# rubiruchi/ofdm_uhd

Hardware: AMD Instinct MI355X
Metric: OFDM symbols/sec (TX+loopback RX) @ N_fft=512; packet CRC pass rate (higher is better)
Workload: dtype f32; 1 GPU; N_fft=512, occ=200, QPSK, CP=128, synthetic AWGN channel (BASELINE configs[1]); payload_bytes=1026, symbols_per_packet=22, streams=1, iq_buffers=1, parallelism=independent streams, 1 per GPU

## Files before the change

ofdm_uhd_amd/csrc/engine_rx.inc:

```

template <typename T>
static int dev_excl_scan(ofdm_handle* h, const T* d_in, uint64_t n, T* d_out, T* d_total) {
  const uint64_t nb = (n + SCAN_BLOCK - 1) / SCAN_BLOCK;
  HIPCHK(h, h->rx.partial.ensure(sizeof(T) * std::max<uint64_t>(nb, 1)));
  T* part = h->rx.partial.as<T>();
  if (n == 0) {
    if (d_total) HIPCHK(h, hipMemsetAsync(d_total, 0, sizeof(T), h->stream));
    return OFDM_OK;
  }
  hipLaunchKernelGGL(HIP_KERNEL_NAME(k_scan_partials<T>), dim3((unsigned)nb), dim3(256), 0, h->stream, d_in, n, part);
  hipLaunchKernelGGL(HIP_KERNEL_NAME(k_scan_top<T>), dim3(1), dim3(256), 0, h->stream, part, nb, d_total);
  hipLaunchKernelGGL(HIP_KERNEL_NAME(k_scan_final<T>), dim3((unsigned)nb), dim3(256), 0, h->stream, d_in, n, part, d_out);
  HIPCHK(h, hipGetLastError());
  return OFDM_OK;
}

template <int N, bool TWL, bool TAPS, bool CSI = false>
static int launch_demod_t(ofdm_handle* h, const DemodParams& q, size_t shmem) {
  constexpr int T = N / 8, FPW = demod_fpw(N);
  if (shmem > 64 * 1024)
    HIPCHK(h, hipFuncSetAttribute(reinterpret_cast<const void*>(&k_rx_demod<N, TWL, TAPS, CSI>),
                                  hipFuncAttributeMaxDynamicSharedMemorySize, (int)shmem));
  hipLaunchKernelGGL(HIP_KERNEL_NAME(k_rx_demod<N, TWL, TAPS, CSI>), dim3((q.nframes + FPW - 1) / FPW), dim3(T * FPW), shmem,
                     h->stream, q);
  HIPCHK(h, hipGetLastError());
  return OFDM_OK;
}
template <int N, bool TWL>
static int launch_demod_v(ofdm_handle* h, const DemodParams& q, size_t shmem) {
  if (q.csi_eq) return launch_demod_t<N, TWL, true, true>(h, q, shmem);
  const bool instr = q.tap_mode != 0 || q.tap_sampler || q.tap_fft || q.tap_acq || q.tap_sink || q.tap_demapped || q.qual;
  return instr ? launch_demod_t<N, TWL, true>(h, q, shmem) : launch_demod_t<N, TWL, false>(h, q, shmem);
}

template <int N>
static int launch_demod(ofdm_handle* h, const DemodParams& q0) {
  DemodParams q = q0;
  constexpr int T = N / 8, WAVES = demod_fpw(N) * ((T + WAVE - 1) / WAVE);
  const bool grid = q.grid != nullptr;
  const bool csi = q.csi_eq != nullptr;
  auto bytes = [&](bool twl, bool sm) {
    return (size_t)demod_lds_bytes(N, twl, sm, q.occ, q.arity, q.nmap, q.nbits, q.shift, grid, csi);
  };
  constexpr int CU_WAVES = 4 * demod_waves_per_simd(N);
  auto wgs = [&](size_t b) { return std::max<size_t>(1, std::min<size_t>(std::max(1, CU_WAVES / WAVES), CU_LDS_BYTES / b)); };
  constexpr bool base_twl = !fft_onebuf(N);
  const size_t w0 = wgs(bytes(base_twl, false));
  bool twl = base_twl;
  if constexpr (fft_onebuf(N)) twl = wgs(bytes(true, false)) == w0 && bytes(true, false) <= CU_LDS_BYTES;
  q.smap_lds = (wgs(bytes(twl, true)) == w0 && bytes(twl, true) <= CU_LDS_BYTES) ? 1 : 0;
  if (const char* e = getenv("OFDM_DEMOD_LDS")) {
    const int v = atoi(e);
    if constexpr (fft_onebuf(N)) twl = (v & 1) != 0;
    q.smap_lds = (v >> 1) & 1;
  }
  const size_t shmem = bytes(twl, q.smap_lds != 0);
  if (shmem > CU_LDS_BYTES) FAIL(h, OFDM_E_INVAL, "configuration needs more than 160 KiB of LDS in k_rx_demod");
  if constexpr (fft_onebuf(N)) {
    return twl ? launch_demod_v<N, true>(h, q, shmem) : launch_demod_v<N, false>(h, q, shmem);
  } else {
    return launch_demod_v<N, true>(h, q, shmem);
  }
}

static int run_demod(ofdm_handle* h, const DemodParams& q) {
  switch (h->N) {
    case 64: return launch_demod<64>(h, q);
    case 128: return launch_demod<128>(h, q);
    case 256: return launch_demod<256>(h, q);
    case 512: return launch_demod<512>(h, q);
    case 1024: return launch_demod<1024>(h, q);
    case 2048: return launch_demod<2048>(h, q);
    default: return launch_demod<4096>(h, q);
  }
}

enum { CT_CAND = 0, CT_OVERFLOW = 1, CT_NLO = 2, CT_NHI = 3, CT_CHAIN = 4, CT_NPEAKS = 5, CT_NSYM = 6, CT_KEYTOT = 7,
       CT_DEFR = 8 , CT_RAWTOT = 13, CT_PIECES = 14, CT_STASH = 15, CT_RECS = 16, CT_COUNT = 17 };

static int sync_params(ofdm_handle* h, uint64_t nsamples, bool cap_full, SyncParams* out) {
  RxState& rx = h->rx;
  const int N = h->N, CP = h->CP, T = SYNC_TILE;
  const uint64_t ntiles = (nsamples + T - 1) / T;
  const int tiles_per_seg = 32 * ((N + CP + T - 1) / T);
  const uint64_t egrid = std::min<uint64_t>(ntiles, 256ull * 8ull), egrid_small = std::min<uint64_t>(ntiles, 256ull * 16ull);
  const uint64_t cand_cap = (cap_full ? nsamples + nsamples / 8 : nsamples / 16) + (egrid + 16) * SYNC_CHUNK_C + egrid_small * 2048ull;
  const uint64_t piece_cap = (cap_full ? nsamples / 2 + 1 : nsamples / 128) + (egrid + egrid_small + 16) * SYNC_CHUNK_P;
  HIPCHK(h, rx.y.ensure(nsamples * sizeof(c32)));
  HIPCHK(h, rx.tile_B.ensure(ntiles * sizeof(double)));
  HIPCHK(h, rx.tile_np.ensure(ntiles * sizeof(uint32_t)));
  HIPCHK(h, rx.tile_pieces.ensure(piece_cap * sizeof(SyncPiece)));
  HIPCHK(h, rx.tile_first.ensure(ntiles * sizeof(uint64_t)));
  HIPCHK(h, rx.avg_in.ensure(ntiles * sizeof(double)));
  HIPCHK(h, rx.cand_u.ensure(cand_cap * sizeof(float)));
  HIPCHK(h, rx.cand_P.ensure(cand_cap * sizeof(c32)));
  HIPCHK(h, rx.counters.ensure(CT_COUNT * sizeof(uint64_t)));
  HIPCHK(h, rx.counts.ensure(ntiles * sizeof(uint32_t)));
  HIPCHK(h, rx.offsets.ensure(ntiles * sizeof(uint32_t)));
  HIPCHK(h, rx.recs.ensure(ntiles * sizeof(SyncRec)));
  float *d_metric = nullptr, *d_presel = nullptr;
  if (h->tap_mask & (1u << OFDM_TAP_RX_METRIC)) {
    HIPCHK(h, rx.metric.ensure(nsamples * sizeof(float)));
    d_metric = rx.metric.as<float>();
  }
  if (h->tap_mask & (1u << OFDM_TAP_RX_PRESEL)) {
    HIPCHK(h, rx.presel.ensure(nsamples * sizeof(float)));
    d_presel = rx.presel.as<float>();
  }
  uint64_t* ctr = rx.counters.as<uint64_t>();
  SyncParams sp;
  memset(&sp, 0, sizeof(sp));
  sp.N = N;
  sp.D = N / 2;
  sp.CP = CP;
  sp.HY = (N + 7) / 8 * 8;
  sp.HM = CP;
  sp.R = sync_ring_samples(sp.HY);
  sp.tiles_per_seg = tiles_per_seg;
  sp.nsamples = nsamples;
  sp.ntiles = ntiles;
  sp.tapcp = (float)(1.0 / (double)CP);
  sp.cand_thr = -fmaxf(h->cfg.peak_rise, h->cfg.peak_fall);
  sp.alpha = h->cfg.peak_alpha;
  sp.decay = (double)(1.0f - h->cfg.peak_alpha);
  sp.y = rx.y.as<c32>();
  sp.metric_tap = d_metric;
  sp.presel_tap = d_presel;
  sp.dpow = h->d_synctab.as<double>();
  sp.ipow = sp.dpow + (SYNC_TILE + 1);
  sp.wtab = reinterpret_cast<const float*>(sp.ipow + (SYNC_TILE + 1));
  sp.tile_B = rx.tile_B.as<double>();
  sp.tile_npieces = rx.tile_np.as<uint32_t>();
  sp.tile_first = rx.tile_first.as<uint64_t>();
  sp.pieces = rx.tile_pieces.as<SyncPiece>();
  sp.piece_cap = piece_cap;
  sp.piece_count = reinterpret_cast<unsigned long long*>(ctr + CT_PIECES);
  sp.cand_u = rx.cand_u.as<float>();
  sp.cand_P = rx.cand_P.as<c32>();
  sp.cand_cap = cand_cap;
  sp.cand_count = reinterpret_cast<unsigned long long*>(ctr + CT_CAND);
  sp.overflow = reinterpret_cast<unsigned int*>(ctr + CT_OVERFLOW);
  sp.recs = rx.recs.as<SyncRec>();
  sp.rec_count = reinterpret_cast<unsigned long long*>(ctr + CT_RECS);
  sp.exact_small = sync_exact_small(CP, N / 2);
  if (const char* es = getenv("OFDM_EXACT_SMALL")) sp.exact_small = std::max(0, std::min(atoi(es), (int)SYNC_TILE));
#ifdef SYNC_DIAG
  if (const char* ab = getenv("OFDM_ABLATE")) sp.ablate = atoi(ab);
#endif
  if (sp.HM > T) FAIL(h, OFDM_E_INVAL, "cyclic prefix longer than a k_sync tile");
  *out = sp;
  return OFDM_OK;
}

static uint64_t sync_nseg(const SyncParams& sp) { return (sp.ntiles + (uint64_t)sp.tiles_per_seg - 1) / (uint64_t)sp.tiles_per_seg; }

#ifdef SYNC_STAMPS
static DevBuf g_stamp_buf;
static int stamps_prepare(ofdm_handle* h, SyncParams& sp, uint64_t nseg) {
  HIPCHK(h, g_stamp_buf.ensure(nseg * 16 * sizeof(unsigned long long)));
  HIPCHK(h, hipMemsetAsync(g_stamp_buf.p, 0, nseg * 16 * sizeof(unsigned long long), h->stream));
  sp.stamps = g_stamp_buf.as<unsigned long long>();
  return OFDM_OK;
}
static int sync_stamps_report(ofdm_handle* h, const unsigned long long* d_stamps, uint64_t nseg, int tiles_per_seg) {
  HIPCHK(h, hipStreamSynchronize(h->stream));
  std::vector<unsigned long long> st(nseg * 16);
  HIPCHK(h, hipMemcpy(st.data(), d_stamps, st.size() * 8, hipMemcpyDeviceToHost));
  double sum[16] = {0};
  for (uint64_t i = 0; i < nseg; i++)
    for (int k = 0; k < 16; k++) sum[k] += (double)st[i * 16 + k];
  const char* nm[16] = {"-", "y tile -> ring / filter", "B2 wait", "terms", "scan3 (B3)", "M + B4", "mavg + B5", "summary", "filter: block A", "filter: block B", "filter: taps + windows in", "-", "-", "-", "-", "-"};
  double tot = 0;
  for (int k = 0; k < 16; k++) tot += sum[k];
  fprintf(stderr, "[k_sync stamps] %llu workgroups, s_memtime ticks per workgroup-tile (wave 0):\n", (unsigned long long)nseg);
  for (int k = 0; k < 11; k++)
    fprintf(stderr, "  %-26s %10.0f  %5.1f%%\n", nm[k], sum[k] / (double)nseg / (double)(tiles_per_seg + 1), 100.0 * sum[k] / tot);
  return OFDM_OK;
}
#endif

static bool front_fused(const ofdm_handle* h) {
  if (h->cfg.sync_mode != OFDM_SYNC_PN) return false;
  const char* e = getenv("OFDM_FRONT");
  if (!e || atoi(e) == 0) return false;
  const int F = h->filtF, B = F - (int)h->cfg.ntaps + 1;
  if (F > 512) return false;
  const int HY = (h->N + 7) / 8 * 8, C = (B + 7) / 8 * 8;
  if (HY + C > SYNC_TILE || h->CP > SYNC_TILE) return false;
  return front_lds_layout(sync_ring_samples(HY), h->CP, B, F).total <= CU_LDS_BYTES / 3;
}

static int launch_sync(ofdm_handle* h, SyncParams& sp) {
  RxState& rx = h->rx;
  const int T = SYNC_TILE;
  const uint64_t nseg = sync_nseg(sp);
  HIPCHK(h, hipMemsetAsync(rx.counters.p, 0, CT_COUNT * sizeof(uint64_t), h->stream));
#ifdef SYNC_STAMPS
  if (int rs = stamps_prepare(h, sp, nseg)) return rs;
#endif
  const size_t sync_shmem = sync_lds_layout(sp.R, sp.HM).total;
  if (sync_shmem > CU_LDS_BYTES) FAIL(h, OFDM_E_INVAL, "configuration needs more than 160 KiB of LDS in k_sync");
  {
    ProfScope span(h->prof, OFDM_K_SYNC, h->stream);
    int wg = (int)std::min<size_t>(SYNC_MAX_WG, CU_LDS_BYTES / sync_shmem);
    if (const char* w = getenv("OFDM_SYNC_W")) wg = std::min(wg, atoi(w));
    bool fixed_layout = sp.R - (int)T <= (int)T;
    if (const char* e = getenv("OFDM_SYNC_STATIC")) fixed_layout = fixed_layout && (atoi(e) != 0 || sync_mt_overlay(sp.R));
    const void* fn = fixed_layout ? (wg >= 6   ? reinterpret_cast<const void*>(&k_sync<6, true>)
                                     : wg == 5 ? reinterpret_cast<const void*>(&k_sync<5, true>)
                                     : wg == 4 ? reinterpret_cast<const void*>(&k_sync<4, true>)
                                     : wg == 3 ? reinterpret_cast<const void*>(&k_sync<3, true>)
                                               : reinterpret_cast<const void*>(&k_sync<2, true>))
                                  : (wg >= 4   ? reinterpret_cast<const void*>(&k_sync<4, false>)
                                     : wg == 3 ? reinterpret_cast<const void*>(&k_sync<3, false>)
                                               : reinterpret_cast<const void*>(&k_sync<2, false>));
    HIPCHK(h, hipFuncSetAttribute(fn, hipFuncAttributeMaxDynamicSharedMemorySize, (int)sync_shmem));
    FilterParams nofp;
    memset(&nofp, 0, sizeof(nofp));
    void* args[] = {&sp, &nofp};
    HIPCHK(h, hipLaunchKernel(fn, dim3((unsigned)nseg), dim3(SYNC_THREADS), args, sync_shmem, h->stream));
  }
  HIPCHK(h, hipGetLastError());
  return OFDM_OK;
}

static void rx_note_input(ofdm_handle* h, const ofdm_c32* iq, uint64_t nsamples) {
  std::swap(h->ev_rx_in, h->ev_rx_in_old);
  h->rx_in_old_pending = h->rx_in_pending;
  h->rx_in_lo[1] = h->rx_in_lo[0];
  h->rx_in_hi[1] = h->rx_in_hi[0];
  h->rx_in_lo[0] = (uintptr_t)iq;
  h->rx_in_hi[0] = (uintptr_t)iq + nsamples * rx_ss(h);
}

static int launch_front(ofdm_handle* h, FilterParams& fp, uint64_t nsamples) {
  const int F = h->filtF;
  SyncParams sp;
  int rcs = sync_params(h, nsamples, false, &sp);
  if (rcs != OFDM_OK) return rcs;
  HIPCHK(h, hipMemsetAsync(h->rx.counters.p, 0, CT_COUNT * sizeof(uint64_t), h->stream));
  const size_t shm = front_lds_layout(sp.R, sp.HM, fp.B, F).total;
  const uint64_t nseg = sync_nseg(sp);
  const void* fn = F == 64    ? reinterpret_cast<const void*>(&k_sync<3, true, 64>)
                   : F == 128 ? reinterpret_cast<const void*>(&k_sync<3, true, 128>)
                   : F == 256 ? reinterpret_cast<const void*>(&k_sync<3, true, 256>)
                              : reinterpret_cast<const void*>(&k_sync<3, true, 512>);
  HIPCHK(h, hipFuncSetAttribute(fn, hipFuncAttributeMaxDynamicSharedMemorySize, (int)shm));
#ifdef SYNC_STAMPS
  if (int rs = stamps_prepare(h, sp, nseg)) return rs;
#endif
  void* args[] = {&sp, &fp};
  {
    ProfScope span(h->prof, OFDM_K_FRONT, h->stream);
    HIPCHK(h, hipLaunchKernel(fn, dim3((unsigned)nseg), dim3(SYNC_THREADS), args, shm, h->stream));
  }
  HIPCHK(h, hipGetLastError());
#ifdef SYNC_STAMPS
  if (int rs = sync_stamps_report(h, sp.stamps, nseg, sp.tiles_per_seg)) return rs;
#endif
  h->rx.front_done = true;
  return OFDM_OK;
}

template <typename XT>
static int launch_filter_t(ofdm_handle* h, FilterParams& fp, uint64_t nsamples) {
  const int F = h->filtF;
  const uint64_t bpr = 256 / (F / 8);
  const uint64_t nblk = (nsamples + (uint64_t)fp.goff + (uint64_t)fp.B - 1) / (uint64_t)fp.B;
  fp.nrounds = (nblk + bpr - 1) / bpr;
  const size_t fsh = (size_t)256 * 9 * sizeof(c32);
  const unsigned fgrid = (unsigned)std::min<uint64_t>(fp.nrounds, 256ull * 8ull * 4ull);
  {
    ProfScope span(h->prof, OFDM_K_FILTER, h->stream);
    switch (F) {
      case 64: hipLaunchKernelGGL(HIP_KERNEL_NAME(k_chan_filter<64, XT>), dim3(fgrid), dim3(256), fsh, h->stream, fp); break;
      case 128: hipLaunchKernelGGL(HIP_KERNEL_NAME(k_chan_filter<128, XT>), dim3(fgrid), dim3(256), fsh, h->stream, fp); break;
      case 256: hipLaunchKernelGGL(HIP_KERNEL_NAME(k_chan_filter<256, XT>), dim3(fgrid), dim3(256), fsh, h->stream, fp); break;
      case 512: hipLaunchKernelGGL(HIP_KERNEL_NAME(k_chan_filter<512, XT>), dim3(fgrid), dim3(256), fsh, h->stream, fp); break;
      case 1024: hipLaunchKernelGGL(HIP_KERNEL_NAME(k_chan_filter<1024, XT>), dim3(fgrid), dim3(256), fsh, h->stream, fp); break;
      default: FAIL(h, OFDM_E_INVAL, "unsupported channel filter transform length");
    }
  }
  HIPCHK(h, hipGetLastError());
  return OFDM_OK;
}

static int launch_filter(ofdm_handle* h, FilterParams& fp, uint64_t nsamples) {
  return h->rx_fmt == OFDM_IQ_SC16 ? launch_filter_t<sc16>(h, fp, nsamples) : launch_filter_t<c32>(h, fp, nsamples);
}

static int rx_submit_impl(ofdm_handle* h, const ofdm_c32* iq, uint64_t nsamples, const c32** d_x_out) {
  RxState& rx = h->rx;
  HIPCHK(h, hipSetDevice(h->cfg.device_id));
  if (h->tx_pending && h->txs != h->stream) HIPCHK(h, hipStreamWaitEvent(h->stream, h->ev_tx_done, 0));
  h->tx_pending = false;
  const c32* d_x = reinterpret_cast<const c32*>(iq);
  if (h->rx_fmt == OFDM_IQ_SC16) {
    if ((uintptr_t)iq & 3u) FAIL(h, OFDM_E_INVAL, "ofdm_sc16 buffers must be 4-byte aligned");
    if (front_fused(h)) FAIL(h, OFDM_E_INVAL, "the fused front end (OFDM_FRONT=1) takes float32 samples only");
  }
  if (!h->dev_ptrs) {
    HIPCHK(h, rx.x_stage.ensure(nsamples * rx_ss(h)));
    HIPCHK(h, hipMemcpyAsync(rx.x_stage.p, iq, nsamples * rx_ss(h), hipMemcpyHostToDevice, h->stream));
    d_x = rx.x_stage.as<c32>();
  }
  *d_x_out = d_x;
  rx.in_event_at_end = true;
  if (h->cfg.sync_mode != OFDM_SYNC_PN) return OFDM_OK;
  HIPCHK(h, rx.y.ensure(nsamples * sizeof(c32)));
  FilterParams fp;
  memset(&fp, 0, sizeof(fp));
  fp.B = h->filtF - (int)h->cfg.ntaps + 1;
  fp.ntm1 = (int)h->cfg.ntaps - 1;
  fp.goff = (int)(rx.origin % (uint64_t)fp.B);
  fp.nsamples = nsamples;
  fp.x = d_x;
  fp.y = rx.y.as<c32>();
  fp.Hf = h->d_Hf.as<c32>();
  fp.twF = h->d_twF.as<c32>();
  fp.xscale = h->rx_scale;
  rx.front_done = false;
  if (int rc = front_fused(h) ? launch_front(h, fp, nsamples) : launch_filter(h, fp, nsamples)) return rc;
  if (!h->sense.rx_on) {
    rx_note_input(h, iq, nsamples);
    HIPCHK(h, hipEventRecord(h->ev_rx_in, h->stream));
    h->rx_in_pending = true;
    rx.in_event_at_end = false;
  }
  return OFDM_OK;
}

extern "C" int ofdm_rx_submit(ofdm_handle* h, const ofdm_c32* iq, uint64_t nsamples) {
  if (!h) return OFDM_E_INVAL;
  if (nsamples && !iq) FAIL(h, OFDM_E_INVAL, "null argument");
  RxState& rx = h->rx;
  rx.sub_valid = false;
  if (nsamples == 0) return OFDM_OK;
  const c32* d_x = nullptr;
  int rc = rx_submit_impl(h, iq, nsamples, &d_x);
  if (rc != OFDM_OK) return rc;
  rx.sub_valid = true;
  rx.sub_iq = iq;
  rx.sub_n = nsamples;
  rx.sub_dx = d_x;
  rx.sub_hold = rx.in_event_at_end;
  return OFDM_OK;
}

struct RxCall {
  ofdm_handle* h;
  const ofdm_c32* iq;
  uint64_t nsamples;
  uint8_t* payload_out;
  uint64_t payload_cap;
  uint64_t* payload_off;
  uint32_t* payload_len;
  uint8_t* crc_ok;
  int max_pkts;
  int* npkt;
  ofdm_stats* stats;
  const c32* d_x = nullptr;
  bool fixed = false;
  bool done = false;
  bool dyn = false;
  uint64_t npeaks = 0, nforced = 0;
  uint64_t n_lo = 0, nframes = 0, nsym = 0, npk = 0, nbytes = 0, rawtot = 0;
  uint64_t npk_ub = 0;
  DynFrames dynf;
  DemodParams dq;
  DeframeParams fq;
  CsiRows csi_fr = {nullptr, nullptr, nullptr, nullptr};
  uint8_t* d_pay = nullptr;
};

static uint64_t* rx_ctr(ofdm_handle* h) { return h->rx.counters.as<uint64_t>(); }

static int rx_read_counts(RxCall& c) {
  ofdm_handle* h = c.h;
  RxState& rx = h->rx;
  uint64_t hc[CT_COUNT];
  HIPCHK(h, hipMemcpyAsync(hc, rx.counters.p, sizeof(hc), hipMemcpyDeviceToHost, h->stream));
  HIPCHK(h, hipStreamSynchronize(h->stream));
  c.n_lo = hc[CT_NLO] & 0xFFFFFFFFull;
  c.nframes = c.npeaks - c.n_lo - (hc[CT_NHI] & 0xFFFFFFFFull);
  c.nsym = hc[CT_NSYM];
  c.npk = hc[CT_KEYTOT] >> 40;
  c.nbytes = hc[CT_KEYTOT] & ((1ull << 40) - 1);
  c.rawtot = hc[CT_RAWTOT];
  rx.nframes = c.nframes;
  rx.j0 = c.n_lo;
  rx.nsym_total = c.nsym;
  if (c.stats) {
    c.stats->frames = c.nframes;
    c.stats->symbols = c.nsym;
    c.stats->headers_ok = hc[CT_DEFR + 0];
    c.stats->chained_frames = hc[CT_DEFR + 3];
    c.stats->overflow = hc[CT_OVERFLOW] & 0xFFFFFFFFull;
  }
  return OFDM_OK;
}

static int rx_check_capacity(RxCall& c) {
  if (c.npk <= (uint64_t)c.max_pkts && c.nbytes <= c.payload_cap) return OFDM_OK;
  *c.npkt = (int)std::min<uint64_t>(c.npk, 0x7FFFFFFF);
  FAIL(c.h, OFDM_E_CAPACITY, "payload_out / max_pkts too small for the packets found");
}

static hipError_t launch_sync_exact(const void* fn, unsigned grid, size_t shmem, SyncParams sp, hipStream_t s) {
  void* args[] = {&sp};
  return hipLaunchKernel(fn, dim3(grid), dim3(SYNC_THREADS), args, shmem, s);
}

static int rx_sync_exact(RxCall& c, SyncParams& sp, bool cap_full) {
  ofdm_handle* h = c.h;
  if (cap_full) {
    int rcs = sync_params(h, c.nsamples, true, &sp);
    if (rcs != OFDM_OK) return rcs;
    uint64_t* ctr = rx_ctr(h);
    HIPCHK(h, hipMemsetAsync(ctr + CT_CAND, 0, 2 * sizeof(uint64_t), h->stream));
    HIPCHK(h, hipMemsetAsync(ctr + CT_NPEAKS, 0, sizeof(uint64_t), h->stream));
    HIPCHK(h, hipMemsetAsync(ctr + CT_PIECES, 0, 2 * sizeof(uint64_t), h->stream));
  }
  const unsigned egrid = (unsigned)std::min<uint64_t>(sp.ntiles, 256ull * 8ull);
  const unsigned egrid_small = (unsigned)std::min<uint64_t>(sp.ntiles, 256ull * 16ull);
  {
    ProfScope span(h->prof, OFDM_K_EXACT, h->stream);
    const size_t esh = exact_lds_layout(sp.CP, SYNC_TILE).total, esh_small = exact_lds_layout(sp.CP, sp.exact_small).total;
    const void* fbig = sp.D >= 2048 ? reinterpret_cast<const void*>(&k_sync_exact<SYNC_THREADS, true>)
                                    : reinterpret_cast<const void*>(&k_sync_exact<SYNC_THREADS, false>);
    if (esh > 64 * 1024) HIPCHK(h, hipFuncSetAttribute(fbig, hipFuncAttributeMaxDynamicSharedMemorySize, (int)esh));
    if (sp.exact_small > 0)
      hipLaunchKernelGGL(HIP_KERNEL_NAME(k_sync_exact<WAVE, false>), dim3(egrid_small), dim3(WAVE), esh_small, h->stream, sp);
    HIPCHK(h, launch_sync_exact(fbig, egrid, esh, sp, h->stream));
    if (sp.metric_tap) {
      SyncParams tp = sp;
      tp.tap_only = 1;
      HIPCHK(h, launch_sync_exact(fbig, egrid, esh, tp, h->stream));
    }
  }
  HIPCHK(h, hipGetLastError());
#ifdef SYNC_STAMPS
  if (!h->rx.front_done)
    if (int rs = sync_stamps_report(h, sp.stamps, sync_nseg(sp), sp.tiles_per_seg)) return rs;
#endif
  return OFDM_OK;
}

static int rx_sense_fork(RxCall& c) {
  ofdm_handle* h = c.h;
  SenseState& ss = h->sense;
  HIPCHK(h, hipEventRecord(ss.ev_in, h->stream));
  HIPCHK(h, hipStreamWaitEvent(ss.side, ss.ev_in, 0));
  int src = sense_enqueue(h, &ss.rx_cfg, c.d_x, c.nsamples, ss.side);
  if (src != OFDM_OK) return src;
  HIPCHK(h, hipEventRecord(ss.ev_out, ss.side));
  return OFDM_OK;
}

static PeakParams make_peak_params(ofdm_handle* h, const SyncParams& sp) {
  RxState& rx = h->rx;
  PeakParams pp;
  memset(&pp, 0, sizeof(pp));
  pp.ntiles = sp.ntiles;
  pp.nsamples = sp.nsamples;
  pp.rise = h->cfg.peak_rise;
  pp.fall = h->cfg.peak_fall;
  pp.alpha = h->cfg.peak_alpha;
  pp.dpow = sp.dpow;
  pp.tile_npieces = rx.tile_np.as<uint32_t>();
  pp.tile_first = rx.tile_first.as<uint64_t>();
  pp.pieces = rx.tile_pieces.as<SyncPiece>();
  pp.avg_in = rx.avg_in.as<double>();
  pp.cand_u = rx.cand_u.as<float>();
  pp.cand_P = rx.cand_P.as<c32>();
  pp.counts = rx.counts.as<uint32_t>();
  pp.offsets = rx.offsets.as<uint32_t>();
  pp.stash_peaks = rx.stash_peaks.as<uint64_t>();
  pp.stash_P = rx.stash_P.as<c32>();
  pp.stash_overflow = reinterpret_cast<unsigned int*>(rx_ctr(h) + CT_STASH);
  if (h->tap_mask & (1u << OFDM_TAP_RX_RUN_AVG)) pp.run_rows = rx.run_rows.as<double>();
  return pp;
}

static int rx_flags_pn(RxCall& c, const SyncParams& sp, uint64_t* overflow) {
  ofdm_handle* h = c.h;
  RxState& rx = h->rx;
  const uint64_t ntiles = sp.ntiles;
  const unsigned grid = (unsigned)((ntiles + 255) / 256);
  uint64_t* ctr = rx_ctr(h);
  const uint64_t run_cap = (h->tap_mask & (1u << OFDM_TAP_RX_RUN_AVG)) ? sp.piece_cap : 0;
  HIPCHK(h, rx.stash_peaks.ensure(ntiles * PEAK_STASH * sizeof(uint64_t)));
  HIPCHK(h, rx.stash_P.ensure(ntiles * PEAK_STASH * sizeof(c32)));
  if (run_cap) HIPCHK(h, rx.run_rows.ensure(run_cap * 2 * sizeof(double)));
  PeakParams pp = make_peak_params(h, sp);
  hipLaunchKernelGGL(k_avg_carry, dim3(grid), dim3(256), 0, h->stream, rx.tile_B.as<double>(), ntiles, c.nsamples, sp.dpow,
                     rx.avg_in.as<double>());
  if (run_cap) HIPCHK(h, hipMemsetAsync(rx.run_rows.p, 0xFF, run_cap * 2 * sizeof(double), h->stream));
  hipLaunchKernelGGL(HIP_KERNEL_NAME(k_peak<false>), dim3(grid), dim3(256), 0, h->stream, pp);
  HIPCHK(h, hipGetLastError());
  int rc = dev_excl_scan<uint32_t>(h, rx.counts.as<uint32_t>(), ntiles, rx.offsets.as<uint32_t>(),
                                   reinterpret_cast<uint32_t*>(ctr + CT_NPEAKS));
  if (rc) return rc;
  uint64_t hc[CT_COUNT];
  HIPCHK(h, hipMemcpyAsync(hc, ctr, sizeof(hc), hipMemcpyDeviceToHost, h->stream));
  HIPCHK(h, hipStreamSynchronize(h->stream));
  if ((*overflow = hc[CT_OVERFLOW] & 0xFFFFFFFFull)) return OFDM_OK;
  rx.run_slots = std::min<uint64_t>(hc[CT_PIECES], run_cap);
  const uint64_t npeaks = hc[CT_NPEAKS] & 0xFFFFFFFFull;
  c.npeaks = rx.npeaks = npeaks;
  if (c.stats) c.stats->peaks = npeaks;
  if (npeaks == 0 && !(rx.nco_ref_on && !rx.hist_flags.empty())) {
    c.done = true;
    return OFDM_OK;
  }
  HIPCHK(h, rx.peaks.ensure(std::max<uint64_t>(npeaks, 1) * sizeof(uint64_t)));
  HIPCHK(h, rx.peak_P.ensure(std::max<uint64_t>(npeaks, 1) * sizeof(c32)));
  pp.peaks = rx.peaks.as<uint64_t>();
  pp.peak_P = rx.peak_P.as<c32>();
  if (npeaks > 0) {
    if (hc[CT_STASH] & 0xFFFFFFFFull)
      hipLaunchKernelGGL(HIP_KERNEL_NAME(k_peak<true>), dim3(grid), dim3(256), 0, h->stream, pp);
    else
      hipLaunchKernelGGL(k_peak_compact, dim3(grid), dim3(256), 0, h->stream, pp);
    HIPCHK(h, hipGetLastError());
  }
  return OFDM_OK;
}

__global__ void __launch_bounds__(256) k_fixed_flags(uint64_t npeaks, uint64_t first, uint64_t period, uint64_t* __restrict__ peaks,
                                                      c32* __restrict__ peak_P) {
  const uint64_t k = (uint64_t)blockIdx.x * blockDim.x + threadIdx.x;
  if (k >= npeaks) return;
  peaks[k] = first + k * period;
  peak_P[k] = mk(0.f, 0.f);
}

static int rx_fixed_count(RxCall& c) {
  ofdm_handle* h = c.h;
  RxState& rx = h->rx;
  const uint64_t L = (uint64_t)h->L;
  c.npeaks = rx.npeaks = c.nsamples >= L ? (c.nsamples - L) / ((uint64_t)h->cfg.fixed_nsymbols * L) + 1 : 0;
  if (c.stats) c.stats->peaks = c.npeaks;
  HIPCHK(h, rx.counters.ensure(CT_COUNT * sizeof(uint64_t)));
  HIPCHK(h, hipMemsetAsync(rx.counters.p, 0, CT_COUNT * sizeof(uint64_t), h->stream));
  if (c.npeaks == 0) {
    HIPCHK(h, hipStreamSynchronize(h->stream));
    c.done = true;
  }
  return OFDM_OK;
}

static int rx_flags_fixed(RxCall& c) {
  ofdm_handle* h = c.h;
  RxState& rx = h->rx;
  HIPCHK(h, rx.peaks.ensure(c.npeaks * sizeof(uint64_t)));
  HIPCHK(h, rx.peak_P.ensure(c.npeaks * sizeof(c32)));
  hipLaunchKernelGGL(k_fixed_flags, dim3((unsigned)((c.npeaks + 255) / 256)), dim3(256), 0, h->stream, c.npeaks, (uint64_t)h->L - 1,
                     (uint64_t)h->cfg.fixed_nsymbols * (uint64_t)h->L, rx.peaks.as<uint64_t>(), rx.peak_P.as<c32>());
  HIPCHK(h, hipGetLastError());
  return OFDM_OK;
}

static int rx_splice(RxCall& c) {
  ofdm_handle* h = c.h;
  RxState& rx = h->rx;
  if (!rx.nco_ref_on) return OFDM_OK;
  const uint64_t npeaks = c.npeaks;
  std::vector<uint64_t> hp(npeaks);
  if (npeaks) HIPCHK(h, hipMemcpyAsync(hp.data(), rx.peaks.p, npeaks * sizeof(uint64_t), hipMemcpyDeviceToHost, h->stream));
  HIPCHK(h, hipStreamSynchronize(h->stream));
  uint64_t kdrop = 0;
  while (kdrop < npeaks && (int64_t)hp[kdrop] <= rx.nco_trust_after) kdrop++;
  const uint64_t m = rx.hist_flags.size(), np2 = m + npeaks - kdrop;
  c.done = np2 == 0;
// ... 823 lines not shown
```

ofdm_uhd_amd/csrc/rx_sync.h:

```cpp
#pragma once
#include "common.h"
#include "fft.h"

#ifndef SYNC_THREADS
#define SYNC_THREADS 256
#endif
#define SYNC_V 8
#define SYNC_TILE (SYNC_THREADS * SYNC_V)
#define SYNC_GUARD 1.0e-3f
#define SYNC_ILL 0.015625f
#define SYNC_CHUNK_C 4096
#ifndef SYNC_MAX_WG
#define SYNC_MAX_WG 5
#endif
#define SYNC_CHUNK_P 1024

struct SyncPiece {
  uint64_t start;
  uint64_t end;
  uint64_t val_off;
  double bloc;
};

struct SyncRec {
  uint64_t tile;
  int amin, bmax;
  float gpre, gpost;
};

struct SyncParams {
  int N, D, CP;
  int HY;
  int HM;
  int R;
  int tiles_per_seg;
  int tap_only;
  int ablate;
  unsigned long long* stamps;
  uint64_t nsamples, ntiles;
  float tapcp;
  float cand_thr;
  float alpha;
  double decay;
  const c32* y;
  float* metric_tap;
  float* presel_tap;
  const double* dpow;
  const double* ipow;
  const float* wtab;
  double* tile_B;
  uint32_t* tile_npieces;
  uint64_t* tile_first;
  SyncPiece* pieces;
  uint64_t piece_cap;
  unsigned long long* piece_count;
  float* cand_u;
  c32* cand_P;
  uint64_t cand_cap;
  unsigned long long* cand_count;
  unsigned int* overflow;
  int exact_small;
  SyncRec* recs;
  unsigned long long* rec_count;
};

__host__ __device__ inline int sync_lp(int i) { return i + (i >> 3); }

__host__ __device__ inline int sync_filter_F(int ntaps) {
  int p2 = 1;
  while (p2 < ntaps) p2 <<= 1;
  const int f = 2 * p2;
  return f < 64 ? 64 : f;
}
__host__ __device__ inline int sync_ring_samples(int HY) { return (HY + SYNC_TILE + 7) / 8 * 8; }

struct FilterParams {
  int B;
  int ntm1;
  int goff;
  uint64_t nsamples, nrounds;
  const c32* x;
  c32* y;
  const c32* Hf;
  const c32* twF;
  float xscale;
};

#ifndef FILTER_W
#define FILTER_W 4
#endif
#ifndef FILTER_PK
#define FILTER_PK true
#endif
template <int F, typename XT = c32>
__global__ void __launch_bounds__(256, FILTER_W) k_chan_filter(FilterParams p) {
  constexpr int TF = F / 8;
  constexpr int BPR = 256 / TF;
  extern __shared__ __align__(16) unsigned char smem[];
  const int tid = threadIdx.x;
  const int g = tid / TF, t = tid % TF;
  c32* sc = reinterpret_cast<c32*>(smem) + g * fft_lds_points(F);
  const int B = p.B, ntm1 = p.ntm1;
  FftTwRegs<F> twr;
  twr.load(p.twF, t);
  c32 Hr[8];
#pragma unroll
  for (int m = 0; m < 8; m++) Hr[m] = p.Hf[t + m * TF];
  auto interior = [&](uint64_t rr) -> bool {
    const int64_t lo = (int64_t)(rr * BPR * (uint64_t)B) - p.goff - ntm1;
    const int64_t hi = (int64_t)((rr * BPR + BPR - 1) * (uint64_t)B) - p.goff + B;
    return lo >= 0 && (uint64_t)hi <= p.nsamples;
  };
  auto load_window = [&](c32 (&xn)[8], uint64_t rr) {
    const int64_t x0 = (int64_t)((rr * BPR + (uint64_t)g) * (uint64_t)B) - p.goff - ntm1 + t;
    if constexpr (std::is_same<XT, c32>::value) {
      if (interior(rr)) {
        const c32* px = p.x + x0;
#pragma unroll
        for (int m = 0; m < 8; m++) xn[m] = px[m * TF];
      } else {
#pragma unroll
        for (int m = 0; m < 8; m++) {
          const int64_t xi = x0 + m * TF;
          xn[m] = (xi >= 0 && (uint64_t)xi < p.nsamples) ? p.x[xi] : mk(0.f, 0.f);
        }
      }
    } else {
      const XT* xs = reinterpret_cast<const XT*>(p.x);
      if (interior(rr)) {
        const XT* px = xs + x0;
#pragma unroll
        for (int m = 0; m < 8; m++) xn[m] = iq_load(px, m * TF, p.xscale);
      } else {
#pragma unroll
        for (int m = 0; m < 8; m++) {
          const int64_t xi = x0 + m * TF;
          xn[m] = (xi >= 0 && (uint64_t)xi < p.nsamples) ? iq_load(xs, xi, p.xscale) : mk(0.f, 0.f);
        }
      }
    }
  };
  auto do_round = [&](c32 (&e)[8], uint64_t r) {
    int tt = t;
    asm volatile("" : "+v"(tt));
    if constexpr (TF <= WAVE) {
      fft_run1<F, false, FILTER_PK>(e, tt, sc, twr, FftWaveSync());
    } else {
      fft_run1<F, false, FILTER_PK>(e, tt, sc, twr, FftBlockSync());
    }
#pragma unroll
    for (int m = 0; m < 8; m++) e[m] = cmul(e[m], Hr[m]);
    asm volatile("" : "+v"(tt));
    if constexpr (TF <= WAVE) {
      fft_run1<F, true, FILTER_PK>(e, tt, sc, twr, FftWaveSync());
    } else {
      fft_run1<F, true, FILTER_PK>(e, tt, sc, twr, FftBlockSync());
    }
    const int64_t bs = (int64_t)((r * BPR + (uint64_t)g) * (uint64_t)B) - p.goff;
    if (interior(r)) {
      c32* py = p.y + (bs + (t - ntm1));
#pragma unroll
      for (int m = 0; m < 8; m++)
        if (t + m * TF >= ntm1) py[m * TF] = e[m];
    } else {
#pragma unroll
      for (int m = 0; m < 8; m++) {
        const int64_t n = bs + (t + m * TF - ntm1);
        if (t + m * TF >= ntm1 && n >= 0 && (uint64_t)n < p.nsamples) p.y[n] = e[m];
      }
    }
  };
  c32 xa[8], xb[8];
  uint64_t r = blockIdx.x;
  const uint64_t stride = gridDim.x;
  if (r < p.nrounds) load_window(xa, r);
  for (; r < p.nrounds; r += 2 * stride) {
    if (r + stride < p.nrounds) load_window(xb, r + stride);
    do_round(xa, r);
    if (r + stride < p.nrounds) {
      if (r + 2 * stride < p.nrounds) load_window(xa, r + 2 * stride);
      do_round(xb, r + stride);
    }
  }
}

struct SyncLds {
  size_t ys, mt, mh, mh1, misc, total;
};
__host__ __device__ inline bool sync_mt_overlay(int R) { return R - SYNC_TILE <= 1000 && R - SYNC_TILE <= SYNC_TILE; }
__host__ __device__ inline SyncLds sync_lds_layout(int R, int HM) {
  SyncLds l;
  size_t o = 0;
  l.ys = o;
  o += (size_t)(sync_lp(R) + 2) * sizeof(c32);
  o = (o + 15) & ~(size_t)15;
  if (sync_mt_overlay(R)) {
    l.mt = l.ys + (size_t)sync_lp(R - SYNC_TILE) * sizeof(c32);
  } else {
    l.mt = o;
    o += ((size_t)(sync_lp(SYNC_TILE) + 2) * sizeof(float) + 15) & ~(size_t)15;
  }
  l.mh = o;
  o += ((size_t)(sync_lp(HM) + 2) * sizeof(float) + 15) & ~(size_t)15;
  l.mh1 = o;
  o += ((size_t)(sync_lp(HM) + 2) * sizeof(float) + 15) & ~(size_t)15;
  l.misc = o;
  o += 384;
  l.total = o;
  return l;
}
struct FrontLds {
  size_t ys, mt, mh0, mh1, tw, misc, total;
  int C;
};
__host__ __device__ inline FrontLds front_lds_layout(int R, int HM, int B, int F) {
  FrontLds l;
  l.C = (B + 7) / 8 * 8;
  size_t o = 0;
  l.ys = o;
  o += (size_t)(sync_lp(R + l.C) + 2) * sizeof(c32);
  o = (o + 15) & ~(size_t)15;
  l.mt = o;
  const size_t mtb = ((size_t)(sync_lp(SYNC_TILE) + 2) * sizeof(float) + 15) & ~(size_t)15;
  const size_t scb = (size_t)SYNC_THREADS * 9 * sizeof(c32);
  o += mtb > scb ? mtb : scb;
  l.mh0 = o;
  o += ((size_t)(sync_lp(HM) + 2) * sizeof(float) + 15) & ~(size_t)15;
  l.mh1 = o;
  o += ((size_t)(sync_lp(HM) + 2) * sizeof(float) + 15) & ~(size_t)15;
  l.tw = o;
  o += ((size_t)fft_tw_lds_points(F) * sizeof(c32) + 15) & ~(size_t)15;
  l.misc = o;
  o += 384;
  l.total = o;
  return l;
}
struct ExactLds {
  size_t me, ue, misc, total;
};
__host__ __device__ inline ExactLds exact_lds_layout(int CP, int rmax) {
  ExactLds l;
  size_t o = 0;
  l.me = o;
  o += ((size_t)(rmax + CP + 8) * sizeof(float) + 15) & ~(size_t)15;
  l.ue = o;
  o += ((size_t)(rmax + 8) * sizeof(float) + 15) & ~(size_t)15;
  l.misc = o;
  o += 512;
  l.total = o;
  return l;
}

__device__ __forceinline__ int ring_wrap(int s, int R) {
  s += (s < 0) ? R : 0;
  s -= (s >= R) ? R : 0;
  return s;
}

struct Aff {
  double A, b;
};
__device__ __forceinline__ Aff aff_then(Aff f, Aff g) {
  Aff r;
  r.A = f.A * g.A;
  r.b = f.b * g.A + g.b;
  return r;
}

template <int CTRL, int ROW_MASK>
__device__ __forceinline__ float dpp_f(float v) {
  return __builtin_bit_cast(float, __builtin_amdgcn_update_dpp(0, __builtin_bit_cast(int, v), CTRL, ROW_MASK, 0xF, false));
}
__device__ __forceinline__ float wave_incl_scan_f32(float v) {
  v += dpp_f<0x111, 0xF>(v);
  v += dpp_f<0x112, 0xF>(v);
  v += dpp_f<0x114, 0xF>(v);
  v += dpp_f<0x118, 0xF>(v);
  v += dpp_f<0x142, 0xA>(v);
  v += dpp_f<0x143, 0xC>(v);
  return v;
}

struct F3 {
  float a, b, c;
};

#define DPP_STEP3(CTRL, MASK)                                                        \
  "v_add_f32_dpp %0, %0, %0 " CTRL " row_mask:" MASK " bank_mask:0xf\n\t"          \
  "v_add_f32_dpp %1, %1, %1 " CTRL " row_mask:" MASK " bank_mask:0xf\n\t"          \
  "v_add_f32_dpp %2, %2, %2 " CTRL " row_mask:" MASK " bank_mask:0xf\n\t"
__device__ __forceinline__ void wave_incl_scan3_f32(float& a, float& b, float& c) {
  asm volatile("s_nop 1\n\t" DPP_STEP3("row_shr:1", "0xf") DPP_STEP3("row_shr:2", "0xf") DPP_STEP3("row_shr:4", "0xf")
                   DPP_STEP3("row_shr:8", "0xf") DPP_STEP3("row_bcast:15", "0xa") DPP_STEP3("row_bcast:31", "0xc")
               : "+v"(a), "+v"(b), "+v"(c));
}
#define DPP_STEP2(CTRL, MASK)                                                        \
  "v_add_f32_dpp %0, %0, %0 " CTRL " row_mask:" MASK " bank_mask:0xf\n\t"          \
  "v_add_f32_dpp %1, %1, %1 " CTRL " row_mask:" MASK " bank_mask:0xf\n\t"          \
  "s_nop 0\n\t"
__device__ __forceinline__ void wave_incl_scan2_f32(float& a, float& b) {
  asm volatile("s_nop 1\n\t" DPP_STEP2("row_shr:1", "0xf") DPP_STEP2("row_shr:2", "0xf") DPP_STEP2("row_shr:4", "0xf")
                   DPP_STEP2("row_shr:8", "0xf") DPP_STEP2("row_bcast:15", "0xa") DPP_STEP2("row_bcast:31", "0xc")
               : "+v"(a), "+v"(b));
}
#define DPP_MAX1(CTRL, MASK) "v_max_f32_dpp %0, %0, %0 " CTRL " row_mask:" MASK " bank_mask:0xf\n\ts_nop 1\n\t"
__device__ __forceinline__ float wave_incl_scanmax_f32(float a) {
  asm volatile("s_nop 1\n\t" DPP_MAX1("row_shr:1", "0xf") DPP_MAX1("row_shr:2", "0xf") DPP_MAX1("row_shr:4", "0xf")
                   DPP_MAX1("row_shr:8", "0xf") DPP_MAX1("row_bcast:15", "0xa") DPP_MAX1("row_bcast:31", "0xc")
               : "+v"(a));
  return a;
}
#define DPP_STEP1(CTRL, MASK) "v_add_f32_dpp %0, %0, %0 " CTRL " row_mask:" MASK " bank_mask:0xf\n\ts_nop 1\n\t"
__device__ __forceinline__ float wave_incl_scan1_f32(float a) {
  asm volatile("s_nop 1\n\t" DPP_STEP1("row_shr:1", "0xf") DPP_STEP1("row_shr:2", "0xf") DPP_STEP1("row_shr:4", "0xf")
                   DPP_STEP1("row_shr:8", "0xf") DPP_STEP1("row_bcast:15", "0xa") DPP_STEP1("row_bcast:31", "0xc")
               : "+v"(a));
  return a;
}

__device__ __forceinline__ void block_scan3_sum3(F3 v, F3 s, float* scratch, F3* excl, F3* sum) {
  const int lane = lane_id(), w = wave_id();
  F3 inc = v, rs = s;
  wave_incl_scan3_f32(inc.a, inc.b, inc.c);
  wave_incl_scan3_f32(rs.a, rs.b, rs.c);
  if (lane == WAVE - 1) {
    scratch[w * 6 + 0] = inc.a;
    scratch[w * 6 + 1] = inc.b;
    scratch[w * 6 + 2] = inc.c;
    scratch[w * 6 + 3] = rs.a;
    scratch[w * 6 + 4] = rs.b;
    scratch[w * 6 + 5] = rs.c;
  }
  __syncthreads();
  F3 base = {0.f, 0.f, 0.f}, sm = {0.f, 0.f, 0.f};
#pragma unroll
  for (int i = 0; i < SYNC_THREADS / WAVE; i++) {
    if (i < w) {
      base.a += scratch[i * 6 + 0];
      base.b += scratch[i * 6 + 1];
      base.c += scratch[i * 6 + 2];
    }
    sm.a += scratch[i * 6 + 3];
    sm.b += scratch[i * 6 + 4];
    sm.c += scratch[i * 6 + 5];
  }
  excl->a = base.a + inc.a - v.a;
  excl->b = base.b + inc.b - v.b;
  excl->c = base.c + inc.c - v.c;
  *sum = sm;
}
__device__ __forceinline__ void block_scan1_sum1(float v, float s, float* scratch, float* excl, float* sum) {
  const int lane = lane_id(), w = wave_id();
  float inc = v, rs = s;
  wave_incl_scan2_f32(inc, rs);
  if (lane == WAVE - 1) {
    scratch[w * 2 + 0] = inc;
    scratch[w * 2 + 1] = rs;
  }
  __syncthreads();
  float base = 0.f, sm = 0.f;
#pragma unroll
  for (int i = 0; i < SYNC_THREADS / WAVE; i++) {
    if (i < w) base += scratch[i * 2 + 0];
    sm += scratch[i * 2 + 1];
  }
  *excl = base + inc - v;
  *sum = sm;
}

struct Q3 {
  long long pr, pi, r;
};

template <int NT>
__device__ __forceinline__ void block_scan3_sum3_i64(Q3 v, Q3 s, long long* scratch, Q3* excl, Q3* sum) {
  const int lane = lane_id(), w = wave_id();
  Q3 inc = v, rs = s;
#pragma unroll
  for (int d = 1; d < WAVE; d <<= 1) {
    const long long a = __shfl_up(inc.pr, d, WAVE), b = __shfl_up(inc.pi, d, WAVE), c = __shfl_up(inc.r, d, WAVE);
    if (lane >= d) {
      inc.pr += a;
      inc.pi += b;
      inc.r += c;
    }
  }
#pragma unroll
  for (int d = WAVE / 2; d > 0; d >>= 1) {
    rs.pr += __shfl_xor(rs.pr, d, WAVE);
    rs.pi += __shfl_xor(rs.pi, d, WAVE);
    rs.r += __shfl_xor(rs.r, d, WAVE);
  }
  if (lane == WAVE - 1) {
    scratch[w * 6 + 0] = inc.pr;
    scratch[w * 6 + 1] = inc.pi;
    scratch[w * 6 + 2] = inc.r;
    scratch[w * 6 + 3] = rs.pr;
    scratch[w * 6 + 4] = rs.pi;
    scratch[w * 6 + 5] = rs.r;
  }
  __syncthreads();
  Q3 base = {0, 0, 0}, sm = {0, 0, 0};
#pragma unroll
  for (int i = 0; i < NT / WAVE; i++) {
    if (i < w) {
      base.pr += scratch[i * 6 + 0];
      base.pi += scratch[i * 6 + 1];
      base.r += scratch[i * 6 + 2];
    }
    sm.pr += scratch[i * 6 + 3];
    sm.pi += scratch[i * 6 + 4];
    sm.r += scratch[i * 6 + 5];
  }
  __syncthreads();
  excl->pr = base.pr + inc.pr - v.pr;
  excl->pi = base.pi + inc.pi - v.pi;
  excl->r = base.r + inc.r - v.r;
  *sum = sm;
}

template <int NT, bool KEEP>
__device__ __forceinline__ void sync_exact_range(const c32* __restrict__ y, float* me, float* ue, c32* gP, float* gU, long long* sc_i64,
                                                 int amin, int bmax, int D, int CP, int64_t t0s, float tapcp) {
  const int tid = threadIdx.x;
  auto ldy = [&](int m) -> c32 {
    const int64_t ia = t0s + (int64_t)m;
    return ia >= 0 ? y[ia] : mk(0.f, 0.f);
  };
  auto qterm = [&](c32 a_, c32 d_) -> Q3 {
    const c32 c_ = cmul_conj(a_, d_);
    Q3 q_;
    q_.pr = q40_clamped(c_.re);
    q_.pi = q40_clamped(c_.im);
    q_.r = q40_clamped(a_.re * a_.re + a_.im * a_.im);
    return q_;
  };
  constexpr int EXACT_G = 4;
  const int s0 = amin - CP;
  const int n_e = bmax - s0;
  const int len = bmax - amin + 1;
  Q3 an = {0, 0, 0};
  for (int m0 = s0 - D + 1 + tid; m0 <= s0; m0 += EXACT_G * NT) {
    c32 ya[EXACT_G], yd[EXACT_G];
#pragma unroll
    for (int u = 0; u < EXACT_G; u++) {
      const int m = m0 + u * NT;
      const bool on = m <= s0;
      ya[u] = on ? ldy(m) : mk(0.f, 0.f);
      yd[u] = on ? ldy(m - D) : mk(0.f, 0.f);
    }
#pragma unroll
    for (int u = 0; u < EXACT_G; u++) {
      if (m0 + u * NT <= s0) {
        const Q3 q = qterm(ya[u], yd[u]);
        an.pr += q.pr;
        an.pi += q.pi;
        an.r += q.r;
      }
    }
  }
  const int lc = (n_e + NT - 1) / NT;
  const int k0 = tid * lc, k1 = (k0 + lc < n_e) ? (k0 + lc) : n_e;
  auto deltas = [&](int k, Q3* d) {
    c32 ya[EXACT_G], yd[EXACT_G], ydd[EXACT_G];
#pragma unroll
    for (int u = 0; u < EXACT_G; u++) {
      const int m = s0 + 1 + k + u;
      const bool on = k + u < k1;
      ya[u] = on ? ldy(m) : mk(0.f, 0.f);
      yd[u] = on ? ldy(m - D) : mk(0.f, 0.f);
      ydd[u] = on ? ldy(m - 2 * D) : mk(0.f, 0.f);
    }
#pragma unroll
    for (int u = 0; u < EXACT_G; u++) {
      const Q3 a = qterm(ya[u], yd[u]), b = qterm(yd[u], ydd[u]);
      d[u].pr = a.pr - b.pr;
      d[u].pi = a.pi - b.pi;
      d[u].r = a.r - b.r;
    }
  };
#ifndef EXACT_KEEP_N
#define EXACT_KEEP_N 12
#endif
  constexpr int EXACT_KEEP = KEEP ? EXACT_KEEP_N : EXACT_G;
// ... 888 lines not shown
```

Measured before the change: 136.4 million OFDM symbols/s.

## Split channel filter rounds into bounds-free interior pipeline and guarded edge loop

Restructures the channel-filter kernel's persistent loop. Each block precomputes the range of rounds that lie fully inside the sample buffer. It runs those rounds in a double-buffered load/transform/store pipeline with pointer increments and no per-round interior checks or 64-bit index recomputation, and adds a scheduling barrier after the loads. Edge rounds go to a separate guarded loop. An environment override for the filter grid size is also added for tuning. The gain depends on how much of the filter cost came from index arithmetic and branching, and the new pipeline adds index-range logic that could be wrong at the edges.

New measurement: 136.8 million OFDM symbols/s, median of 6. Within noise of the previous version (+0.3%).

```diff
diff --git a/ofdm_uhd_amd/csrc/engine_rx.inc b/ofdm_uhd_amd/csrc/engine_rx.inc
--- a/ofdm_uhd_amd/csrc/engine_rx.inc
+++ b/ofdm_uhd_amd/csrc/engine_rx.inc
@@ -269,7 +269,10 @@
   const uint64_t nblk = (nsamples + (uint64_t)fp.goff + (uint64_t)fp.B - 1) / (uint64_t)fp.B;
   fp.nrounds = (nblk + bpr - 1) / bpr;
   const size_t fsh = (size_t)256 * 9 * sizeof(c32);
-  const unsigned fgrid = (unsigned)std::min<uint64_t>(fp.nrounds, 256ull * 8ull * 4ull);
+  unsigned fgrid = (unsigned)std::min<uint64_t>(fp.nrounds, 256ull * 8ull * 4ull);
+  if (const char* e = getenv("OFDM_FILTER_GRID")) {
+    if (fgrid) fgrid = (unsigned)std::max(1, std::min(atoi(e), (int)fgrid));
+  }
   {
     ProfScope span(h->prof, OFDM_K_FILTER, h->stream);
     switch (F) {
diff --git a/ofdm_uhd_amd/csrc/rx_sync.h b/ofdm_uhd_amd/csrc/rx_sync.h
--- a/ofdm_uhd_amd/csrc/rx_sync.h
+++ b/ofdm_uhd_amd/csrc/rx_sync.h
@@ -106,41 +106,16 @@
   c32 Hr[8];
 #pragma unroll
   for (int m = 0; m < 8; m++) Hr[m] = p.Hf[t + m * TF];
-  auto interior = [&](uint64_t rr) -> bool {
-    const int64_t lo = (int64_t)(rr * BPR * (uint64_t)B) - p.goff - ntm1;
-    const int64_t hi = (int64_t)((rr * BPR + BPR - 1) * (uint64_t)B) - p.goff + B;
-    return lo >= 0 && (uint64_t)hi <= p.nsamples;
-  };
-  auto load_window = [&](c32 (&xn)[8], uint64_t rr) {
-    const int64_t x0 = (int64_t)((rr * BPR + (uint64_t)g) * (uint64_t)B) - p.goff - ntm1 + t;
-    if constexpr (std::is_same<XT, c32>::value) {
-      if (interior(rr)) {
-        const c32* px = p.x + x0;
-#pragma unroll
-        for (int m = 0; m < 8; m++) xn[m] = px[m * TF];
-      } else {
-#pragma unroll
-        for (int m = 0; m < 8; m++) {
-          const int64_t xi = x0 + m * TF;
-          xn[m] = (xi >= 0 && (uint64_t)xi < p.nsamples) ? p.x[xi] : mk(0.f, 0.f);
-        }
-      }
-    } else {
-      const XT* xs = reinterpret_cast<const XT*>(p.x);
-      if (interior(rr)) {
-        const XT* px = xs + x0;
-#pragma unroll
-        for (int m = 0; m < 8; m++) xn[m] = iq_load(px, m * TF, p.xscale);
-      } else {
-#pragma unroll
-        for (int m = 0; m < 8; m++) {
-          const int64_t xi = x0 + m * TF;
-          xn[m] = (xi >= 0 && (uint64_t)xi < p.nsamples) ? iq_load(xs, xi, p.xscale) : mk(0.f, 0.f);
-        }
-      }
-    }
-  };
-  auto do_round = [&](c32 (&e)[8], uint64_t r) {
+  const uint64_t stride = gridDim.x, r0 = blockIdx.x;
+  const uint64_t RS = (uint64_t)BPR * (uint64_t)B;
+  const uint64_t ilo = ((uint64_t)(p.goff + ntm1) + RS - 1) / RS;
+  const uint64_t ihi = std::max<uint64_t>((p.nsamples + (uint64_t)p.goff) / RS, ilo);
+  auto first_i = [&](uint64_t rr) -> uint64_t { return rr > r0 ? (rr - r0 + stride - 1) / stride : 0; };
+  const uint64_t ia = first_i(ilo), ni = first_i(p.nrounds);
+  const uint64_t ib = first_i(ihi) >= ia + 2 ? first_i(ihi) : ia;
+  auto index_of = [&](uint64_t rr) -> int64_t { return (int64_t)((rr * BPR + (uint64_t)g) * (uint64_t)B) - p.goff - ntm1 + t; };
+  const XT* const xs = reinterpret_cast<const XT*>(p.x);
+  auto transform = [&](c32 (&e)[8]) {
     int tt = t;
     asm volatile("" : "+v"(tt));
     if constexpr (TF <= WAVE) {
@@ -156,30 +131,64 @@
     } else {
       fft_run1<F, true, FILTER_PK>(e, tt, sc, twr, FftBlockSync());
     }
-    const int64_t bs = (int64_t)((r * BPR + (uint64_t)g) * (uint64_t)B) - p.goff;
-    if (interior(r)) {
-      c32* py = p.y + (bs + (t - ntm1));
+  };
+
+  if (ia < ib) {
+    const int64_t s0 = (int64_t)((r0 + ia * stride) * RS) - p.goff - ntm1;
+    const int64_t adv = (int64_t)(stride * RS);
+    const int voff = g * B + t;
+    const XT* px = xs + s0 + voff;
+    c32* py = p.y + s0 + voff;
+    auto load = [&](c32 (&w)[8]) {
+#pragma unroll
+      for (int m = 0; m < 8; m++) w[m] = iq_load(px, m * TF, p.xscale);
+      px += adv;
+      __builtin_amdgcn_sched_barrier(0);
+    };
+    auto store = [&](const c32 (&e)[8]) {
 #pragma unroll
       for (int m = 0; m < 8; m++)
         if (t + m * TF >= ntm1) py[m * TF] = e[m];
-    } else {
-#pragma unroll
-      for (int m = 0; m < 8; m++) {
-        const int64_t n = bs + (t + m * TF - ntm1);
-        if (t + m * TF >= ntm1 && n >= 0 && (uint64_t)n < p.nsamples) p.y[n] = e[m];
-      }
-    }
-  };
-  c32 xa[8], xb[8];
-  uint64_t r = blockIdx.x;
-  const uint64_t stride = gridDim.x;
-  if (r < p.nrounds) load_window(xa, r);
-  for (; r < p.nrounds; r += 2 * stride) {
-    if (r + stride < p.nrounds) load_window(xb, r + stride);
-    do_round(xa, r);
-    if (r + stride < p.nrounds) {
-      if (r + 2 * stride < p.nrounds) load_window(xa, r + 2 * stride);
-      do_round(xb, r + stride);
+      py += adv;
+    };
+    c32 xa[8], xb[8];
+    uint64_t unloaded = ib - ia - 2;
+    load(xa);
+    load(xb);
+    transform(xa);
+    store(xa);
+    for (; unloaded >= 2; unloaded -= 2) {
+      load(xa);
+      transform(xb);
+      store(xb);
+      load(xb);
+      transform(xa);
+      store(xa);
+    }
+    if (unloaded) load(xa);
+    transform(xb);
+    store(xb);
+    if (unloaded) {
+      transform(xa);
+      store(xa);
+    }
+  }
+
+  for (uint64_t i = 0; i < ni; i++) {
+    if (i == ia) i = ib;
+    if (i >= ni) break;
+    const int64_t i0 = index_of(r0 + i * stride);
+    c32 e[8];
+#pragma unroll
+    for (int m = 0; m < 8; m++) {
+      const int64_t xi = i0 + m * TF;
+      e[m] = (xi >= 0 && (uint64_t)xi < p.nsamples) ? iq_load(xs, xi, p.xscale) : mk(0.f, 0.f);
+    }
+    transform(e);
+#pragma unroll
+    for (int m = 0; m < 8; m++) {
+      const int64_t n = i0 + m * TF;
+      if (t + m * TF >= ntm1 && n >= 0 && (uint64_t)n < p.nsamples) p.y[n] = e[m];
     }
   }
 }
```
